# scaleoutsystems/fedn

Measured on AMD Instinct MI355X. Metric: aggregated params/sec (device-resident) — FedAvg 64-client reduce, 100M fp32, higher is better.
Workload: dtype f32

## Files before the change

fedn_amd/_abi.py:

```python
import ctypes
import os
import threading

_HERE = os.path.dirname(os.path.abspath(__file__))
LIB_NAME = "libfedagg.so"
LIB_PATH = os.path.join(_HERE, LIB_NAME)

FA_NONE, FA_F32, FA_F64, FA_BF16, FA_F16, FA_I32, FA_I64 = -1, 0, 1, 2, 3, 4, 5
FA_I8, FA_I16, FA_U8, FA_U16, FA_U32, FA_U64 = 6, 7, 8, 9, 10, 11
FA_OK, FA_EINVAL, FA_EDTYPE, FA_EHIP = 0, 1, 2, 3
FA_ADAM, FA_YOGI, FA_ADAGRAD = 0, 1, 2
FA_PG_FIRST, FA_PG_FINAL = 1, 2
(FA_EW_AXPBY, FA_EW_MUL, FA_EW_DIV, FA_EW_SQRT, FA_EW_SQUARE, FA_EW_SIGN, FA_EW_FILL, FA_EW_POW, FA_EW_IPOW, FA_EW_IFOLD,
 FA_EW_NFOLD) = range(11)
(FA_TUNE_STRIPS, FA_TUNE_UNROLL, FA_TUNE_NT, FA_TUNE_FASTDIV, FA_TUNE_LANETAB, FA_TUNE_GRID, FA_TUNE_READ,
 FA_TUNE_BLOCK, FA_TUNE_SUM_NOSTORE, FA_TUNE_NT_STORE, FA_TUNE_FASTDIV64, FA_TUNE_TILEMAP, FA_TUNE_OPT_NT,
 FA_TUNE_OPT_NOSTORE, FA_TUNE_OPT_STORE, FA_TUNE_OPT_COAL, FA_TUNE_NARROW, FA_TUNE_LDS, FA_TUNE_WPE, FA_TUNE_OPT_MV, FA_TUNE_AUTO_GEOM,
 FA_TUNE_OPT_MIX, FA_TUNE_OPT_BURST, FA_TUNE_OPT_G, FA_TUNE_OPT_WIN_PERIOD, FA_TUNE_OPT_WIN_W, FA_TUNE_OPT_WIN_MODE,
 FA_TUNE_AVG_WIN_PERIOD, FA_TUNE_AVG_WIN_W, FA_TUNE_AVG_WIN_MODE, FA_TUNE_OPT_WIN_PROD,
 FA_TUNE_OPT_QUAD) = range(32)

EXPORTS = {
    "fa_abi_version": (ctypes.c_int, []),
    "fa_last_error": (ctypes.c_char_p, []),
    "fa_last_kernel": (ctypes.c_char_p, []),
    "fa_promote": (ctypes.c_int, [ctypes.c_int, ctypes.c_int]),
    "fa_fedavg_fold": (ctypes.c_int, [
        ctypes.c_void_p, ctypes.c_int,
        ctypes.POINTER(ctypes.c_void_p), ctypes.c_int,
        ctypes.POINTER(ctypes.c_double), ctypes.POINTER(ctypes.c_double), ctypes.c_int,
        ctypes.c_int64, ctypes.c_int, ctypes.c_void_p]),
    "fa_fedavg_fold_host": (ctypes.c_int, [
        ctypes.c_void_p, ctypes.c_int,
        ctypes.POINTER(ctypes.c_void_p), ctypes.c_int,
        ctypes.POINTER(ctypes.c_double), ctypes.POINTER(ctypes.c_double), ctypes.c_int,
        ctypes.c_int64, ctypes.c_int, ctypes.c_void_p]),
    "fa_fedopt_step_host": (ctypes.c_int, [
        ctypes.c_void_p, ctypes.c_int,
        ctypes.POINTER(ctypes.c_void_p), ctypes.c_int,
        ctypes.POINTER(ctypes.c_double), ctypes.POINTER(ctypes.c_double), ctypes.c_int,
        ctypes.c_void_p, ctypes.c_int, ctypes.c_void_p, ctypes.c_int,
        ctypes.c_void_p, ctypes.c_int, ctypes.c_void_p, ctypes.c_void_p, ctypes.c_int,
        ctypes.c_int, ctypes.c_double, ctypes.c_double, ctypes.c_double, ctypes.c_double,
        ctypes.c_int64, ctypes.c_void_p]),
    "fa_fedopt_step": (ctypes.c_int, [
        ctypes.c_void_p, ctypes.c_int,
        ctypes.POINTER(ctypes.c_void_p), ctypes.c_int,
        ctypes.POINTER(ctypes.c_double), ctypes.POINTER(ctypes.c_double), ctypes.c_int,
        ctypes.c_void_p, ctypes.c_int,
        ctypes.c_void_p, ctypes.c_int, ctypes.c_void_p,
        ctypes.c_void_p, ctypes.c_void_p, ctypes.c_void_p,
        ctypes.c_int, ctypes.c_double, ctypes.c_double, ctypes.c_double, ctypes.c_double,
        ctypes.c_int64, ctypes.c_void_p]),
    "fa_fedopt_step_ex": (ctypes.c_int, [
        ctypes.c_void_p, ctypes.c_int,
        ctypes.POINTER(ctypes.c_void_p), ctypes.c_int,
        ctypes.POINTER(ctypes.c_double), ctypes.POINTER(ctypes.c_double), ctypes.c_int,
        ctypes.c_void_p, ctypes.c_int,
        ctypes.c_void_p, ctypes.c_int, ctypes.c_void_p, ctypes.c_int,
        ctypes.c_void_p, ctypes.c_int, ctypes.c_void_p, ctypes.c_void_p, ctypes.c_int,
        ctypes.c_int, ctypes.c_double, ctypes.c_double, ctypes.c_double, ctypes.c_double,
        ctypes.c_int64, ctypes.c_void_p]),
    "fa_weighted_sum": (ctypes.c_int, [
        ctypes.c_void_p, ctypes.c_int,
        ctypes.POINTER(ctypes.c_void_p), ctypes.c_int,
        ctypes.POINTER(ctypes.c_double), ctypes.c_int,
        ctypes.c_int64, ctypes.c_void_p]),
    "fa_running_mean": (ctypes.c_int, [
        ctypes.c_void_p, ctypes.c_int, ctypes.c_void_p,
        ctypes.c_double, ctypes.c_double, ctypes.c_double,
        ctypes.c_int64, ctypes.c_void_p]),
    "fa_elementwise": (ctypes.c_int, [ctypes.c_int, ctypes.c_void_p, ctypes.c_int, ctypes.c_void_p, ctypes.c_int,
                                      ctypes.c_void_p, ctypes.c_int, ctypes.c_double, ctypes.c_double, ctypes.c_int64,
# ... 145 lines not shown
```

fedn_amd/build.py:

```python
import os
import shutil
import subprocess
import sys

HERE = os.path.dirname(os.path.abspath(__file__))
ROOT = os.path.dirname(HERE)
SRC = os.path.join(HERE, "csrc", "fedagg.hip")
HDR = os.path.join(ROOT, "include", "fedagg.h")
OUT = os.path.join(HERE, "libfedagg.so")
PROBE_HDR = os.path.join(ROOT, "include", "fedagg_probe.h")
PROBE_OUT = os.path.join(HERE, "libfedagg_probe.so")
ARCH = os.environ.get("FEDN_AMD_ARCH", "gfx950")

FLAGS = ["-O3", "-std=c++17", "-ffp-contract=off", "-fPIC", "-shared", "-Wall", f"--offload-arch={ARCH}"]


def hipcc():
    for cand in (os.environ.get("HIPCC"), shutil.which("hipcc"), "/opt/rocm/bin/hipcc"):
        if cand and os.path.exists(cand):
            return cand
    raise RuntimeError("hipcc not found")


NPZ_SRC = os.path.join(HERE, "csrc", "npz_codec.cpp")
# ... 11 lines not shown

def build_codec(force=False, verbose=True):
    deps = [d for d in (NPZ_SRC, NPZ_HDR, NPZ_INFLATE, NPZ_SAVEZ, NPZ_PDEFLATE, NPZ_GUARD) if os.path.exists(d)]
    if not force and not _stale(NPZ_OUT, *deps):
        return NPZ_OUT
    cxx = os.environ.get("CXX") or shutil.which("g++") or "g++"
    tmp = NPZ_OUT + ".tmp"
    cmd = [cxx, "-O3", "-std=c++17", "-fPIC", "-shared", "-pthread", "-Wall", "-I", os.path.join(ROOT, "include"),
           "-o", tmp, NPZ_SRC, NPZ_SAVEZ, "-lz"]
    if verbose:
        print(" ".join(cmd), flush=True)
    subprocess.run(cmd, check=True)
    os.replace(tmp, NPZ_OUT)
    return NPZ_OUT


FASTPACK_SRC = os.path.join(HERE, "csrc", "fastpack.c")
FASTPACK_OUT = os.path.join(HERE, "_fastpack.so")


def build_fastpack(force=False, verbose=True):
    if not force and not _stale(FASTPACK_OUT, FASTPACK_SRC):
        return FASTPACK_OUT
    import sysconfig

    import numpy
    cc = os.environ.get("CC") or shutil.which("gcc") or "gcc"
    tmp = FASTPACK_OUT + ".tmp"
    cmd = [cc, "-O2", "-fPIC", "-shared", "-Wall", "-I", sysconfig.get_paths()["include"], "-I", numpy.get_include(),
           "-o", tmp, FASTPACK_SRC]
    if verbose:
        print(" ".join(cmd), flush=True)
    subprocess.run(cmd, check=True)
    os.replace(tmp, FASTPACK_OUT)
    return FASTPACK_OUT


def build(force=False, verbose=True):
    from concurrent.futures import ThreadPoolExecutor
    with ThreadPoolExecutor(4) as ex:
        futs = [ex.submit(build_codec, force, verbose), ex.submit(build_hip, force, verbose),
                ex.submit(build_hip, force, verbose, True), ex.submit(build_fastpack, force, verbose)]
        for f in futs:
            f.result()
    return OUT


def build_hip(force=False, verbose=True, probe=False):
    out = PROBE_OUT if probe else OUT
    deps = (SRC, HDR, PROBE_HDR)
    if not force and not _stale(out, *deps):
        return out
    tmp = out + ".tmp"
    cmd = [hipcc()] + FLAGS + (["-DFEDAGG_PROBES"] if probe else []) + ["-I", os.path.join(ROOT, "include"),
                                                                          "-o", tmp, SRC]
    if verbose:
        print(" ".join(cmd), flush=True)
    subprocess.run(cmd, check=True)
    os.replace(tmp, out)
    return out


if __name__ == "__main__":
    print(build(force="--force" in sys.argv), NPZ_OUT)
```

fedn_amd/csrc/fedagg.hip:

```cpp

#include <hip/hip_runtime.h>
#include <hip/hip_fp16.h>

#include <cmath>
#include <cstdarg>
#include <cstdint>
#include <cstdio>
#include <algorithm>
#include <atomic>
#include <cstring>
#include <type_traits>
#include <vector>

#include "../../include/fedagg.h"
#ifdef FEDAGG_PROBES
#include "../../include/fedagg_probe.h"
#endif

namespace {

thread_local char g_err[512] = "";
thread_local const char* g_kernel = "";

int fail(int code, const char* fmt, ...) {
// ... 562 lines not shown
        };
        auto fold = [&](int kk, const Y (&y)[S][E]) {
            const typename CP::S n = LT ? LaneTable<CP>::rl(lt.n, kk) : tab.n[kk];
            const typename CP::S N = LT ? LaneTable<CP>::rl(lt.N, kk) : tab.N[kk];
            const double r = LT ? LaneTable<CP>::rl(lt.r, kk) : tab.r[kk];
#pragma unroll
            for (int s = 0; s < S; ++s) {
                V yv[E];
#pragma unroll
                for (int e = 0; e < E; ++e) yv[e] = widen<Y, V>(y[s][e]);
                fold_strip<CP, E>(x[s], yv, n, N, r);
            }
        };
        Y a[S][E], b[S][E];
        if (k < K) load(k, a);
        while (k + 1 < K) {
            if constexpr (WIN) {
                if (win_mode >= 2) wait_read_window(period, win_w);
            }
            load(k + 1, b);
            fold(k, a);
            if (k + 2 < K) load(k + 2, a);
            fold(k + 1, b);
            k += 2;
        }
        if (k < K) fold(k, a);
        if constexpr (WIN) wait_write_window(period, win_w);
#pragma unroll
        for (int s = 0; s < S; ++s) {
            X xo[E];
#pragma unroll
            for (int e = 0; e < E; ++e) xo[e] = narrow<X, V>(x[s][e]);
            if constexpr (is_nostore<CP>::value) {
                if (__float_as_uint(x[s][0]) != 0xFFFFFFFFu) continue;
            }
            strip_store<X, E, NTS>(agg + (strip0 + s * BLK) * E, xo);
        }
    }
}

template <typename Y, typename X, class CP, int E, int S, bool INIT, bool INT_FIRST, bool NT, bool LT, int BLK = kBlock,
          int NTS = 0, int MAP = 0>
__global__ void __launch_bounds__(BLK)
k_fedavg_pipe(X* __restrict__ agg, const ClientTable<typename CP::S> tab, const int K, const int64_t P) {
    fedavg_pipe_body<Y, X, CP, E, S, INIT, INT_FIRST, NT, LT, BLK, NTS, MAP>(agg, tab, K, P);
}

template <typename Y, typename X, class CP, int E, int S, bool INIT, bool INT_FIRST, bool NT, bool LT, int BLK, int NTS,
          int MAP>
__global__ void __launch_bounds__(BLK)
k_fedavg_pipe_win(X* __restrict__ agg, const ClientTable<typename CP::S> tab, const int K, const int64_t P,
                  const uint32_t period, const uint32_t win_w, const int win_mode) {
    fedavg_pipe_body<Y, X, CP, E, S, INIT, INT_FIRST, NT, LT, BLK, NTS, MAP, true>(agg, tab, K, P, period, win_w, win_mode);
}

#ifdef FEDAGG_PROBES
template <typename Y, typename X, class CP, int E, int S, bool INIT, bool INT_FIRST, bool NT, bool LT, int BLK, int NTS,
          int MAP, int W>
__global__ void __launch_bounds__(BLK) __attribute__((amdgpu_waves_per_eu(W)))
k_fedavg_pipe_w(X* __restrict__ agg, const ClientTable<typename CP::S> tab, const int K, const int64_t P) {
    fedavg_pipe_body<Y, X, CP, E, S, INIT, INT_FIRST, NT, LT, BLK, NTS, MAP>(agg, tab, K, P);
}
#endif

struct OptScalars {
    double lr, b1, b2, tau, tau2, c1, c2, nc2;
    float b1f, c1f, c2f;
    float b1h, c1h, c2h;
    int opt;
};

struct OptBuffers {
    const void* old;
    void* pg;
    const void* m_in;
    void* m_out;
    const void* v_in;
    void* v_out;
    void* out;
    int m_in_f64;
    int m_out_f64;
    int v_in_f32;
    int v_out_f32;
    int out_f32;
};

template <class PG> __device__ __forceinline__ double mul_pg(double a, double c, float cf, float ch);
template <> __device__ __forceinline__ double mul_pg<CF32>(double a, double, float cf, float) { return (double)((float)a * cf); }
template <> __device__ __forceinline__ double mul_pg<CF64>(double a, double c, float, float) { return a * c; }
template <> __device__ __forceinline__ double mul_pg<CF16>(double a, double, float, float ch) {
    return (double)CF16::rh((float)a * ch);
}

template <class PG> __device__ __forceinline__ typename PG::V pg_sub(typename PG::V y, typename PG::V o) { return y - o; }
template <> __device__ __forceinline__ float pg_sub<CF16>(float y, float o) { return CF16::rh(y - o); }
template <class PG> __device__ __forceinline__ typename PG::V pg_sq(typename PG::V v) { return (typename PG::V)(v * v); }
template <> __device__ __forceinline__ float pg_sq<CF16>(float v) { return CF16::rh(v * v); }

__device__ __forceinline__ double np_sign(double d) {
    return d > 0.0 ? 1.0 : (d < 0.0 ? -1.0 : (d == 0.0 ? 0.0 : d));
}

template <int E, bool SNT = false>
__device__ __forceinline__ void opt_load_state(const OptBuffers& b, const OptScalars& s, int64_t i0, int rem,
                                               double (&mi)[E], double (&v)[E]) {
    const bool full = rem == E;
// ... 971 lines not shown
        for (int j = 0; j < kPushWords; ++j) {
            const int64_t i = base + (int64_t)j * kBlock;
            if (i < n16) v[j] = __builtin_nontemporal_load(src + i);
        }
        for (int d = 0; d < nd; ++d) {
            u32x4* __restrict__ o = t.dst[d];
#pragma unroll
            for (int j = 0; j < kPushWords; ++j) {
                const int64_t i = base + (int64_t)j * kBlock;
                if (i < n16) __builtin_nontemporal_store(v[j], o + i);
            }
        }
    }
}

__global__ void k_push_tail(PushTable t, int nd, const uint8_t* __restrict__ src, int64_t off, int rem) {
    const int b = threadIdx.x;
    if (b < rem)
        for (int d = 0; d < nd; ++d) reinterpret_cast<uint8_t*>(t.dst[d])[off + b] = src[off + b];
}

#ifdef FEDAGG_PROBES
__global__ void __launch_bounds__(kBlock) k_stream_copy(u32x4* __restrict__ dst, const u32x4* __restrict__ src, int64_t n16) {
    const int64_t i = (int64_t)blockIdx.x * kBlock + threadIdx.x;
    if (i < n16) dst[i] = __builtin_nontemporal_load(src + i);
}

constexpr int kReadPerLane = 16;
template <int RPL>
__global__ void __launch_bounds__(kBlock) k_stream_read(const u32x4* __restrict__ src, int64_t n16, u32x4* __restrict__ sink) {
    const int64_t base = (int64_t)blockIdx.x * kBlock * RPL + threadIdx.x;
    u32x4 acc = {0, 0, 0, 0};
#pragma unroll
    for (int j = 0; j < RPL; ++j) {
        const int64_t i = base + (int64_t)j * kBlock;
        if (i < n16) acc ^= __builtin_nontemporal_load(src + i);
    }
    __shared__ u32x4 red[kBlock];
    red[threadIdx.x] = acc;
    __syncthreads();
    if (threadIdx.x == 0) {
        u32x4 r = red[0];
        for (int t = 1; t < kBlock; ++t) r ^= red[t];
        sink[blockIdx.x] = r;
    }
}
#endif

bool aligned16(const void* p) { return (reinterpret_cast<uintptr_t>(p) & 15u) == 0; }

#ifdef FEDAGG_PROBES
struct FedAvgCfg {
    std::atomic<int> strips{4}, unroll{0}, lanetab{0}, grid_per_cu{0}, read_per_lane{16}, block_log{8},
        sum_nostore{0}, nt_store{1}, nt{0}, tilemap{0}, fastdiv{1}, fastdiv64{1}, opt_nt{1}, opt_nostore{0}, opt_store{0}, opt_coal{2}, narrow{1}, lds_kib{0}, wpe{0}, opt_mv{0}, auto_geom{1}, opt_mix{0}, opt_burst{0}, opt_g{0}, opt_win_period{0}, opt_win_w{0}, opt_win_mode{0}, avg_win_period{0}, avg_win_w{0}, avg_win_mode{0}, opt_win_prod{0}, opt_quad{0};
};
FedAvgCfg g_cfg;
int cfg_fastdiv() { return g_cfg.fastdiv.load(std::memory_order_relaxed); }
int cfg_fastdiv64() { return g_cfg.fastdiv64.load(std::memory_order_relaxed); }
int cfg_grid_per_cu() { return g_cfg.grid_per_cu.load(std::memory_order_relaxed); }
#else
constexpr int cfg_fastdiv() { return 1; }
constexpr int cfg_fastdiv64() { return 1; }
constexpr int cfg_grid_per_cu() { return 0; }
#endif

template <typename S>
void fill_table(ClientTable<S>& t, const void* const* ptrs, const double* n, const double* N, int k0, int cnt) {
    for (int j = 0; j < cnt; ++j) {
        t.ptr[j] = ptrs[k0 + j];
        t.n[j] = (S)n[k0 + j];
        t.N[j] = (S)N[k0 + j];
        if constexpr (std::is_same<S, double>::value) {
            const double Nd = N[k0 + j], a = std::fabs(Nd);
            t.r[j] = (cfg_fastdiv64() && a >= 0x1p-60 && a <= 0x1p60) ? 1.0 / Nd : 0.0;
        } else {
            const float Nf = (float)N[k0 + j];
            t.r[j] = (cfg_fastdiv() && Nf != 0.0f && std::fabs(Nf) < 0x1p28f) ? 1.0 / (double)Nf : 0.0;
        }
    }
    for (int j = cnt; j < kMaxK; ++j) {
        t.ptr[j] = nullptr;
        t.n[j] = 0;
        t.N[j] = 0;
        t.r[j] = 0.0;
    }
}

float to_half_value(double v) { return (float)(_Float16)v; }

int64_t grid_for(int64_t P, int E) {
    const int64_t strips = (P + E - 1) / E;
    return (strips + kBlock - 1) / kBlock;
}

int device_cus() {
    int dev = 0, cus = 256;
    if (hipGetDevice(&dev) != hipSuccess ||
        hipDeviceGetAttribute(&cus, hipDeviceAttributeMultiprocessorCount, dev) != hipSuccess)
        cus = 256;
    return cus > 0 ? cus : 256;
}

struct StoreWindow {
    uint32_t period = 0, w = 0;
};
template <typename Y, typename OLD, class PG, bool NT>
StoreWindow opt_store_window(const OptBuffers& b, int K, int64_t P) {
    const bool state = b.m_in_f64 >= 0 || b.v_in;
    if (K < (state ? 32 : 8) || P < ((int64_t)1 << 24)) return {};
    static std::atomic<int> blocks_per_cu{-1};
    int nb = blocks_per_cu.load(std::memory_order_relaxed);
    if (nb < 0) {
        nb = 0;
        if (hipOccupancyMaxActiveBlocksPerMultiprocessor(&nb, k_fedopt_cw<Y, OLD, PG, NT>, kBlock, 0) != hipSuccess) nb = 0;
        blocks_per_cu.store(nb, std::memory_order_relaxed);
    }
    if (nb <= 0) return {};
    const double waves = (double)nb * (kBlock / 64) * device_cus();
    const double m_in = b.m_in_f64 == 1 ? 8 : b.m_in_f64 == 0 ? 4 : b.m_in_f64 < 0 ? 0 : 2;
    const double m_out = b.m_out_f64 == 1 ? 8 : b.m_out_f64 == 0 ? 4 : 2;
    const double rd = (double)K * sizeof(Y) + sizeof(OLD) + m_in + (b.v_in ? (b.v_in_f32 ? 4 : 8) : 0);
    const double wr = (b.out_f32 ? 4 : 8) + (b.v_out_f32 ? 4 : 8) + m_out;
    const double frac = wr / (rd + wr);
    if (frac > 0.25) return {};
    const double period = (state ? 0.35 : 0.65) * waves * 512.0 * (rd + wr) / 6.4e12 * 1e8;
    if (period < 1000 || period > 20000) return {};
    StoreWindow sw;
    sw.period = (uint32_t)period;
    sw.w = (uint32_t)(period * (state ? 0.15 : std::min(0.30, std::max(0.08, 1.15 * frac))));
    return sw;
}


struct AvgWindow {
    uint32_t period = 0, w = 0;
};
template <typename Y, typename X, class CP, int E, int S, bool NT, bool LT, int BLK, int NTS, int MAP>
AvgWindow avg_store_window(int K, int64_t P) {
    if (P < ((int64_t)1 << 24) || K < 2) return {};
    static std::atomic<int> blocks_per_cu{-1};
    int nb = blocks_per_cu.load(std::memory_order_relaxed);
    if (nb < 0) {
        nb = 0;
        if (hipOccupancyMaxActiveBlocksPerMultiprocessor(&nb, k_fedavg_pipe_win<Y, X, CP, E, S, true, false, NT, LT, BLK, NTS, MAP>,
                                                         BLK, 0) != hipSuccess)
            nb = 0;
        blocks_per_cu.store(nb, std::memory_order_relaxed);
    }
    if (nb <= 0) return {};
    if ((double)sizeof(X) / ((double)K * sizeof(Y) + sizeof(X)) > 0.15) return {};
    const double round_bytes = (double)nb * device_cus() * BLK * S * E * ((double)K * sizeof(Y) + sizeof(X));
    const double period = 0.45 * round_bytes / 6.4e12 * 1e8;
    if (period < 500 || period > 20000) return {};
    AvgWindow w;
    w.period = (uint32_t)period;
    w.w = (uint32_t)(0.15 * period);
    return w;
}

template <typename Y, typename X, class CP, int E, int S, bool NT, bool LT, int BLK = kBlock, int NTS = 0, int MAP = 0>
void launch_fedavg_pipe(X* a, const ClientTable<typename CP::S>& tab, int cnt, int64_t P, bool first, bool int_first,
                        hipStream_t st) {
    g_kernel = "k_fedavg_pipe";
    const int64_t strips = (P + E - 1) / E;
    int64_t ntiles = (strips + (int64_t)BLK * S - 1) / ((int64_t)BLK * S);
    if (cfg_grid_per_cu() > 0) {
        if constexpr (MAP != 0) return launch_fedavg_pipe<Y, X, CP, E, S, NT, LT, BLK, NTS, 0>(a, tab, cnt, P, first, int_first, st);
        ntiles = std::min<int64_t>(ntiles, (int64_t)cfg_grid_per_cu() * device_cus());
    }
    const dim3 grid((unsigned)ntiles);
    unsigned shm = 0;
    if constexpr (std::is_same<CP, CF32>::value && std::is_same<X, float>::value &&
                  ((std::is_same<Y, float>::value && S * E == 16) || (std::is_same<Y, bf16>::value && S * E == 32)) &&
                  BLK == kBlock && MAP == 0 && !LT && !NT && NTS == 1) {
        if (first && !int_first && cfg_grid_per_cu() == 0) {
            AvgWindow w = avg_store_window<Y, X, CP, E, S, NT, LT, BLK, NTS, MAP>(cnt, P);
            int wm = 0;
#ifdef FEDAGG_PROBES
            if (g_cfg.avg_win_period < 0 || g_cfg.wpe > 0 || g_cfg.lds_kib > 0) w = AvgWindow{};
            else if (g_cfg.avg_win_period > 0) {
                w = AvgWindow{(uint32_t)g_cfg.avg_win_period.load(), (uint32_t)g_cfg.avg_win_w.load()};
                wm = g_cfg.avg_win_mode.load();
            }
#endif
            if (w.period) {
                g_kernel = "k_fedavg_pipe_win";
                hipLaunchKernelGGL((k_fedavg_pipe_win<Y, X, CP, E, S, true, false, NT, LT, BLK, NTS, MAP>), grid, dim3(BLK), 0, st, a,
                                   tab, cnt, P, w.period, w.w, wm);
                return;
            }
        }
    }
#ifdef FEDAGG_PROBES
    shm = (unsigned)g_cfg.lds_kib * 1024u;
    if constexpr (std::is_same<CP, CF32>::value && std::is_same<X, float>::value && S * E * (int)sizeof(Y) == 64 &&
                  BLK == kBlock && MAP == 0 && !LT && !NT && NTS == 1) {
        if (g_cfg.avg_win_period > 0 && !int_first && !first) {
            const uint32_t wl = (uint32_t)g_cfg.avg_win_period.load(), ww = (uint32_t)g_cfg.avg_win_w.load();
            g_kernel = "k_fedavg_pipe_win";
            hipLaunchKernelGGL((k_fedavg_pipe_win<Y, X, CP, E, S, false, false, NT, LT, BLK, NTS, MAP>), grid, dim3(BLK), shm, st, a, tab,
                               cnt, P, wl, ww, g_cfg.avg_win_mode.load());
            return;
        }
        const int w = g_cfg.wpe;
        if (w > 0 && !int_first) {
#define FA_WPE(W_)                                                                                                      \
    if (w == W_) {                                                                                                      \
        if (first) hipLaunchKernelGGL((k_fedavg_pipe_w<Y, X, CP, E, S, true, false, NT, LT, BLK, NTS, MAP, W_>), grid, dim3(BLK), shm, st, a, tab, cnt, P); \
        else hipLaunchKernelGGL((k_fedavg_pipe_w<Y, X, CP, E, S, false, false, NT, LT, BLK, NTS, MAP, W_>), grid, dim3(BLK), shm, st, a, tab, cnt, P); \
        return;                                                                                                         \
    }
            FA_WPE(5) FA_WPE(6) FA_WPE(8)
#undef FA_WPE
        }
    }
#endif
    if (first && int_first) {
        if constexpr (std::is_integral<Y>::value)
            hipLaunchKernelGGL((k_fedavg_pipe<Y, X, CP, E, S, true, true, NT, LT, BLK, NTS, MAP>), grid, dim3(BLK), shm, st, a, tab, cnt, P);
    } else if (first)
        hipLaunchKernelGGL((k_fedavg_pipe<Y, X, CP, E, S, true, false, NT, LT, BLK, NTS, MAP>), grid, dim3(BLK), shm, st, a, tab, cnt, P);
    else
        hipLaunchKernelGGL((k_fedavg_pipe<Y, X, CP, E, S, false, false, NT, LT, BLK, NTS, MAP>), grid, dim3(BLK), shm, st, a, tab, cnt, P);
}

template <typename Y, typename X, class CP, int E, int S, int U, bool NT>
void launch_fedavg_geom(X* a, const ClientTable<typename CP::S>& tab, int cnt, int64_t P, bool first, bool int_first,
                        hipStream_t st) {
    g_kernel = "k_fedavg";
    const int64_t strips = (P + E - 1) / E;
    const dim3 grid((unsigned)((strips + (int64_t)kBlock * S - 1) / ((int64_t)kBlock * S)));
    if (first && int_first) {
        if constexpr (std::is_integral<Y>::value)
            hipLaunchKernelGGL((k_fedavg<Y, X, CP, E, S, U, true, true, NT>), grid, dim3(kBlock), 0, st, a, tab, cnt, P);
    } else if (first)
        hipLaunchKernelGGL((k_fedavg<Y, X, CP, E, S, U, true, false, NT>), grid, dim3(kBlock), 0, st, a, tab, cnt, P);
    else
        hipLaunchKernelGGL((k_fedavg<Y, X, CP, E, S, U, false, false, NT>), grid, dim3(kBlock), 0, st, a, tab, cnt, P);
}

constexpr int64_t kPipeMinClientBytes = 160ll << 20;

template <typename Y>
inline bool pipe_pays(int64_t P) { return P * (int64_t)sizeof(Y) >= kPipeMinClientBytes; }

template <typename Y, typename X, class CP, int E>
void launch_fedavg_small(X* a, const ClientTable<typename CP::S>& tab, int cnt, int64_t P, bool first, bool int_first,
                         hipStream_t st);

template <class CP> struct is_sf_rule : std::false_type {};
template <typename Y, typename X> struct is_sf_rule<CWSUM<Y, X>> : std::true_type {};
template <typename T_> struct is_sf_rule<CRUN<T_>> : std::true_type {};
// ... 1005 lines not shown
        case FA_TUNE_AUTO_GEOM:
            g_cfg.auto_geom = value ? 1 : 0;
            return FA_OK;
        case FA_TUNE_OPT_MV:
            g_cfg.opt_mv = value ? 1 : 0;
            return FA_OK;
        case FA_TUNE_OPT_MIX:
            g_cfg.opt_mix = value ? 1 : 0;
            return FA_OK;
        case FA_TUNE_OPT_G:
            if (value != 0 && value != 1 && value != 2 && value != 4)
                return fail(FA_EINVAL, "fa_tune: burst-store product probe 0 (off), 1, 2 or 4 tiles per wave");
            g_cfg.opt_g = value;
            return FA_OK;
        case FA_TUNE_OPT_WIN_PERIOD:
            if (value != 0 && value != -1 && (value < 64 || value > (1 << 24)))
                return fail(FA_EINVAL, "fa_tune: store-window period 64 .. 2^24 ticks of 10 ns (0 = the product's own, -1 = none)");
            g_cfg.opt_win_period = value;
            return FA_OK;
        case FA_TUNE_OPT_WIN_W:
            if (value < 0) return fail(FA_EINVAL, "fa_tune: store-window length in ticks >= 0");
            g_cfg.opt_win_w = value;
            return FA_OK;
        case FA_TUNE_OPT_WIN_MODE:
            if (value < 0 || value > 2) return fail(FA_EINVAL, "fa_tune: store-window mode 0, 1 or 2");
            g_cfg.opt_win_mode = value;
            return FA_OK;
        case FA_TUNE_OPT_WIN_PROD:
            if (value < 0 || value > 3)
                return fail(FA_EINVAL, "fa_tune: OPT_WIN_PROD 0 (pattern probe), 1 (k_fedopt_cw), 2 (k_fedopt_cgw), 3 (k_fedopt_cw2)");
            g_cfg.opt_win_prod = value;
            return FA_OK;
        case FA_TUNE_OPT_QUAD:
            g_cfg.opt_quad = value ? 1 : 0;
            return FA_OK;
        case FA_TUNE_AVG_WIN_PERIOD:
            if (value != 0 && value != -1 && (value < 64 || value > (1 << 24)))
                return fail(FA_EINVAL, "fa_tune: store-window period 64 .. 2^24 ticks of 10 ns (0 = the product's own, -1 = none)");
            g_cfg.avg_win_period = value;
            return FA_OK;
        case FA_TUNE_AVG_WIN_W:
            if (value < 0) return fail(FA_EINVAL, "fa_tune: store-window length in ticks >= 0");
            g_cfg.avg_win_w = value;
            return FA_OK;
        case FA_TUNE_AVG_WIN_MODE:
            if (value < 0 || value > 2) return fail(FA_EINVAL, "fa_tune: store-window mode 0, 1 or 2");
            g_cfg.avg_win_mode = value;
            return FA_OK;
        case FA_TUNE_OPT_BURST:
            if (value != 0 && value != 1 && value != 2 && value != 4)
                return fail(FA_EINVAL, "fa_tune: burst-store probe 0 (off), 1, 2 or 4 tiles per wave");
            g_cfg.opt_burst = value;
            return FA_OK;
        case FA_TUNE_WPE:
            if (value != 0 && value != 5 && value != 6 && value != 7 && value != 8)
                return fail(FA_EINVAL, "fa_tune: waves per SIMD 0 (compiler's choice), 5, 6, 7 or 8");
            g_cfg.wpe = value;
            return FA_OK;
        default:
            return fail(FA_EINVAL, "fa_tune: unknown knob %d", knob);
    }
}

int fa_stream_sum(float* out, const float* const* bufs, int K, int64_t P, void* stream) {
    g_err[0] = 0;
    if (K < 1 || K > kMaxK || P < 0 || !out || !bufs) return fail(FA_EINVAL, "fa_stream_sum: bad arguments");
    bool vec = aligned16(out);
    for (int k = 0; k < K; ++k) vec = vec && bufs[k] && aligned16(bufs[k]);
    if (!vec) return fail(FA_EINVAL, "fa_stream_sum: buffers must be 16-B aligned");
    ClientTable<float> tab;
    std::vector<double> ones(K, 1.0);
    fill_table<float>(tab, reinterpret_cast<const void* const*>(bufs), ones.data(), ones.data(), 0, K);
    if (g_cfg.sum_nostore)
        launch_fedavg_pipe<float, float, CADDNW, 4, 4, false, false>(out, tab, K, P, true, false, static_cast<hipStream_t>(stream));
    else if (g_cfg.nt_store == 1)
        launch_fedavg_pipe<float, float, CADD, 4, 4, false, false, kBlock, 1>(out, tab, K, P, true, false, static_cast<hipStream_t>(stream));
    else if (g_cfg.nt_store == 2)
        launch_fedavg_pipe<float, float, CADD, 4, 4, false, false, kBlock, 2>(out, tab, K, P, true, false, static_cast<hipStream_t>(stream));
    else
        launch_fedavg_pipe<float, float, CADD, 4, 4, false, false>(out, tab, K, P, true, false, static_cast<hipStream_t>(stream));
    return check_launch("fa_stream_sum");
}

int fa_stream_copy(void* dst, const void* src, int64_t bytes, void* stream) {
    g_err[0] = 0;
    if (bytes < 0 || (bytes & 15) || !aligned16(dst) || !aligned16(src))
        return fail(FA_EINVAL, "fa_stream_copy: bytes must be a multiple of 16 and buffers 16-B aligned");
    const int64_t n16 = bytes / 16;
    if (!n16) return FA_OK;
    hipLaunchKernelGGL(k_stream_copy, dim3((unsigned)((n16 + kBlock - 1) / kBlock)), dim3(kBlock), 0,
                       static_cast<hipStream_t>(stream), static_cast<u32x4*>(dst), static_cast<const u32x4*>(src), n16);
    return check_launch("fa_stream_copy");
}

int64_t fa_stream_read_blocks(int64_t bytes) {
    const int64_t n16 = bytes / 16;
    const int64_t per = (int64_t)kBlock * kReadPerLane;
    return (n16 + per - 1) / per;
}

int fa_stream_read(const void* src, int64_t bytes, void* sink, void* stream) {
    g_err[0] = 0;
    if (bytes < 0 || (bytes & 15) || !aligned16(src) || !aligned16(sink))
        return fail(FA_EINVAL, "fa_stream_read: bytes must be a multiple of 16 and buffers 16-B aligned");
    const int64_t blocks = fa_stream_read_blocks(bytes);
    if (!blocks) return FA_OK;
// ... 17 lines not shown
```

fedn_amd/ops.py:

```python
import contextlib
import ctypes

import numpy as np
import torch

from . import _abi
from ._abi import FedAggError

_TORCH_TO_FA = {
    torch.float32: _abi.FA_F32,
    torch.float64: _abi.FA_F64,
    torch.bfloat16: _abi.FA_BF16,
    torch.float16: _abi.FA_F16,
    torch.int32: _abi.FA_I32,
    torch.int64: _abi.FA_I64,
    torch.int8: _abi.FA_I8,
    torch.int16: _abi.FA_I16,
    torch.uint8: _abi.FA_U8,
    torch.uint16: _abi.FA_U16,
    torch.uint32: _abi.FA_U32,
    torch.uint64: _abi.FA_U64,
}
_FA_TO_TORCH = {v: k for k, v in _TORCH_TO_FA.items()}
_NP_TO_TORCH = {
# ... 285 lines not shown
        rc = lib.fa_cast(out.data_ptr(), fa_dtype(out), x.data_ptr(), fa_dtype(x), len(ms), _abi.int64_array(ms),
                         _abi.int64_array(mt), st)
    _abi.check(rc)
    return out


def _probe_lib():
    lib = _abi.load()
    if lib is not _abi._probe:
        raise RuntimeError("measurement / tuning entry point: call fedn_amd._abi.use_probe() first "
                           "(libfedagg_probe.so; the product libfedagg.so has no knobs)")
    return lib


def stream_copy(dst, src, stream=None):
    lib = _probe_lib()
    st = _stream_handle(src, stream)
    _abi.check(lib.fa_stream_copy(dst.data_ptr(), src.data_ptr(), src.numel() * src.element_size(), st))


def stream_sum(out, bufs, stream=None):
    lib = _probe_lib()
    st = _stream_handle(out, stream)
    _abi.check(lib.fa_stream_sum(out.data_ptr(), _abi.ptr_array([b.data_ptr() for b in bufs]), len(bufs),
                                 out.numel(), st))


def stream_read(src, sink, stream=None):
    lib = _probe_lib()
    st = _stream_handle(src, stream)
    _abi.check(lib.fa_stream_read(src.data_ptr(), src.numel() * src.element_size(), sink.data_ptr(), st))


def stream_read_sink(src):
    lib = _probe_lib()
    blocks = lib.fa_stream_read_blocks(src.numel() * src.element_size())
    return torch.empty(max(1, blocks) * 16, dtype=torch.uint8, device=src.device)


_KNOBS = {"strips": _abi.FA_TUNE_STRIPS, "unroll": _abi.FA_TUNE_UNROLL, "nt": _abi.FA_TUNE_NT,
          "fastdiv": _abi.FA_TUNE_FASTDIV, "lanetab": _abi.FA_TUNE_LANETAB,
          "grid": _abi.FA_TUNE_GRID, "read": _abi.FA_TUNE_READ,
          "block": _abi.FA_TUNE_BLOCK, "sum_nostore": _abi.FA_TUNE_SUM_NOSTORE,
          "nt_store": _abi.FA_TUNE_NT_STORE, "fastdiv64": _abi.FA_TUNE_FASTDIV64,
          "tilemap": _abi.FA_TUNE_TILEMAP, "opt_nt": _abi.FA_TUNE_OPT_NT, "opt_nostore": _abi.FA_TUNE_OPT_NOSTORE,
          "opt_store": _abi.FA_TUNE_OPT_STORE, "opt_coal": _abi.FA_TUNE_OPT_COAL, "narrow": _abi.FA_TUNE_NARROW,
          "lds": _abi.FA_TUNE_LDS, "wpe": _abi.FA_TUNE_WPE,
          "opt_mv": _abi.FA_TUNE_OPT_MV, "auto_geom": _abi.FA_TUNE_AUTO_GEOM,
          "opt_mix": _abi.FA_TUNE_OPT_MIX, "opt_burst": _abi.FA_TUNE_OPT_BURST,
          "opt_g": _abi.FA_TUNE_OPT_G, "opt_win_period": _abi.FA_TUNE_OPT_WIN_PERIOD, "opt_win_w": _abi.FA_TUNE_OPT_WIN_W,
          "opt_win_mode": _abi.FA_TUNE_OPT_WIN_MODE, "avg_win_period": _abi.FA_TUNE_AVG_WIN_PERIOD,
          "avg_win_w": _abi.FA_TUNE_AVG_WIN_W, "avg_win_mode": _abi.FA_TUNE_AVG_WIN_MODE,
          "opt_win_prod": _abi.FA_TUNE_OPT_WIN_PROD,
          "opt_quad": _abi.FA_TUNE_OPT_QUAD}


def tune(**knobs):
    lib = _probe_lib()
    for k, v in knobs.items():
        _abi.check(lib.fa_tune(_KNOBS[k], int(v)))


_EW = {"axpby": _abi.FA_EW_AXPBY, "mul": _abi.FA_EW_MUL, "div": _abi.FA_EW_DIV, "sqrt": _abi.FA_EW_SQRT,
       "square": _abi.FA_EW_SQUARE, "sign": _abi.FA_EW_SIGN, "fill": _abi.FA_EW_FILL, "pow": _abi.FA_EW_POW,
       "ipow": _abi.FA_EW_IPOW, "ifold": _abi.FA_EW_IFOLD, "nfold": _abi.FA_EW_NFOLD}


def elementwise(op, out, x=None, y=None, a=0.0, b=0.0, stream=None):
    lib = _abi.load()
    P = out.numel()
    _check_dev("out", out, P, None)
    for name, t in (("x", x), ("y", y)):
        if t is not None:
            _check_dev(name, t, P, out.device)
    if P == 0:
        for t in (out, x, y):
            if t is not None:
                fa_dtype(t)
        if op not in _EW:
            raise ValueError(f"unknown elementwise op {op}")
        return out
    with _on(out.device):
        st = _stream_handle(out, stream)
        rc = lib.fa_elementwise(_EW[op], out.data_ptr(), fa_dtype(out), 0 if x is None else x.data_ptr(),
                                fa_dtype(out) if x is None else fa_dtype(x), 0 if y is None else y.data_ptr(),
                                _abi.FA_NONE if y is None else fa_dtype(y), float(a), float(b), P, st)
    _abi.check(rc)
    return out


def norm1(x, matrix, stream=None):
    lib = _abi.load()
    if not x.is_contiguous():
        raise ValueError("norm1: x must be contiguous")
    rows, cols = (x.shape[0], x.shape[1]) if matrix else (1, x.numel())
    work = torch.empty(max(1, int(lib.fa_norm1_work(rows, cols, int(matrix)))), dtype=torch.float64, device=x.device)
    out = torch.empty((), dtype=torch.float64, device=x.device)
    with _on(x.device):
        st = _stream_handle(x, stream)
        rc = lib.fa_norm1(out.data_ptr(), x.data_ptr(), fa_dtype(x), rows, cols, int(matrix), work.data_ptr(), st)
    _abi.check(rc)
    return out



def ipc_handle(t):
    import ctypes
# ... 167 lines not shown
```

include/fedagg_probe.h:

```cpp
#ifndef FEDAGG_PROBE_H
#define FEDAGG_PROBE_H

#include "fedagg.h"

#ifdef __cplusplus
extern "C" {
#endif

int fa_stream_copy(void* dst, const void* src, int64_t bytes, void* stream);
int fa_stream_sum(float* out, const float* const* bufs, int K, int64_t P, void* stream);

enum fa_tune_knob { FA_TUNE_STRIPS = 0, FA_TUNE_UNROLL = 1, FA_TUNE_NT = 2, FA_TUNE_FASTDIV = 3, FA_TUNE_LANETAB = 4,
                    FA_TUNE_GRID = 5, FA_TUNE_READ = 6 ,
                    FA_TUNE_BLOCK = 7 ,
                    FA_TUNE_SUM_NOSTORE = 8 ,
                    FA_TUNE_NT_STORE = 9 ,
                    FA_TUNE_FASTDIV64 = 10 ,
                    FA_TUNE_TILEMAP = 11 ,
                    FA_TUNE_OPT_NT = 12 ,
                    FA_TUNE_OPT_NOSTORE = 13 ,
                    FA_TUNE_OPT_STORE = 14 ,
                    FA_TUNE_OPT_COAL = 15 ,
                    FA_TUNE_NARROW = 16 ,
                    FA_TUNE_LDS = 17 ,
                    FA_TUNE_WPE = 18 ,
                    FA_TUNE_OPT_MV = 19 ,
                    FA_TUNE_AUTO_GEOM = 20 ,
                    FA_TUNE_OPT_MIX = 21 ,
                    FA_TUNE_OPT_BURST = 22 ,
                    FA_TUNE_OPT_G = 23 ,
                    FA_TUNE_OPT_WIN_PERIOD = 24 ,
                    FA_TUNE_OPT_WIN_W = 25 ,
                    FA_TUNE_OPT_WIN_MODE = 26 ,
                    FA_TUNE_AVG_WIN_PERIOD = 27 ,
                    FA_TUNE_AVG_WIN_W = 28,
                    FA_TUNE_AVG_WIN_MODE = 29,
                    FA_TUNE_OPT_WIN_PROD = 30 ,
                    FA_TUNE_OPT_QUAD = 31  };
int fa_tune(int knob, int value);
int64_t fa_stream_read_blocks(int64_t bytes);
int fa_stream_read(const void* src, int64_t bytes, void* sink, void* stream);

#ifdef __cplusplus
}
#endif

#endif
```

Measured before the change: 1489 billion.

## Add rolling-refill FedAvg fold kernel for large client counts with tuned store window

Adds a new FedAvg fold body that keeps one client's strips in flight and refills each strip's buffer right after folding it, replacing the ping-pong double-buffer body for f32 inputs when K >= 48. The aim is smoother memory-level parallelism and fewer stalls between clients in the bandwidth-bound reduce. The roll kernel uses its own store-window period (a smaller fraction of the round bytes, with a higher cap). The build now also captures compiler kernel-resource remarks into a file, and a probe knob selects the fold body. Risk: different register pressure and occupancy, and a new tuned window heuristic.

```diff
diff --git a/fedn_amd/_abi.py b/fedn_amd/_abi.py
--- a/fedn_amd/_abi.py
+++ b/fedn_amd/_abi.py
@@ -18,7 +18,7 @@
  FA_TUNE_OPT_NOSTORE, FA_TUNE_OPT_STORE, FA_TUNE_OPT_COAL, FA_TUNE_NARROW, FA_TUNE_LDS, FA_TUNE_WPE, FA_TUNE_OPT_MV, FA_TUNE_AUTO_GEOM,
  FA_TUNE_OPT_MIX, FA_TUNE_OPT_BURST, FA_TUNE_OPT_G, FA_TUNE_OPT_WIN_PERIOD, FA_TUNE_OPT_WIN_W, FA_TUNE_OPT_WIN_MODE,
  FA_TUNE_AVG_WIN_PERIOD, FA_TUNE_AVG_WIN_W, FA_TUNE_AVG_WIN_MODE, FA_TUNE_OPT_WIN_PROD,
- FA_TUNE_OPT_QUAD) = range(32)
+ FA_TUNE_OPT_QUAD, FA_TUNE_AVG_BODY) = range(33)
 
 EXPORTS = {
     "fa_abi_version": (ctypes.c_int, []),
diff --git a/fedn_amd/build.py b/fedn_amd/build.py
--- a/fedn_amd/build.py
+++ b/fedn_amd/build.py
@@ -87,14 +87,52 @@
     if not force and not _stale(out, *deps):
         return out
     tmp = out + ".tmp"
-    cmd = [hipcc()] + FLAGS + (["-DFEDAGG_PROBES"] if probe else []) + ["-I", os.path.join(ROOT, "include"),
+    cmd = [hipcc()] + FLAGS + (["-DFEDAGG_PROBES"] if probe else []) + [RESOURCE_FLAG, "-I", os.path.join(ROOT, "include"),
                                                                           "-o", tmp, SRC]
     if verbose:
         print(" ".join(cmd), flush=True)
-    subprocess.run(cmd, check=True)
+    p = subprocess.run(cmd, stderr=subprocess.PIPE, text=True)
+    import re
+    remarks, rest, quoted = [], [], False
+    for line in p.stderr.splitlines(keepends=True):
+        if RESOURCE_FLAG in line:
+            remarks.append(line)
+            quoted = True
+        elif not (quoted and re.match(r"\s*\d*\s*\|", line)):
+            rest.append(line)
+            quoted = False
+    sys.stderr.write("".join(rest))
+    if p.returncode:
+        raise subprocess.CalledProcessError(p.returncode, cmd)
+    with open(resources_path(probe), "w") as f:
+        f.writelines(remarks)
     os.replace(tmp, out)
     return out
 
 
+RESOURCE_FLAG = "-Rpass-analysis=kernel-resource-usage"
+
+
+def resources_path(probe=False):
+    return (PROBE_OUT if probe else OUT) + ".resources.txt"
+
+
+def kernel_resources(text):
+    import re
+    fields = {"VGPRs": "vgprs", "AGPRs": "agprs", "TotalSGPRs": "sgprs", "ScratchSize [bytes/lane]": "scratch",
+              "Occupancy [waves/SIMD]": "occupancy"}
+    res, cur = {}, None
+    for line in text.splitlines():
+        m = re.search(r"remark: (?:\S+: )?\s*([A-Za-z][A-Za-z /\[\]]*?): (\S+) \[" + re.escape(RESOURCE_FLAG), line)
+        if not m:
+            continue
+        key, val = m.group(1).strip(), m.group(2)
+        if key == "Function Name":
+            cur = res.setdefault(val, {})
+        elif cur is not None and key in fields and val.isdigit():
+            cur[fields[key]] = int(val)
+    return res
+
+
 if __name__ == "__main__":
     print(build(force="--force" in sys.argv), NPZ_OUT)
diff --git a/fedn_amd/csrc/fedagg.hip b/fedn_amd/csrc/fedagg.hip
--- a/fedn_amd/csrc/fedagg.hip
+++ b/fedn_amd/csrc/fedagg.hip
@@ -638,6 +638,82 @@
 k_fedavg_pipe_win(X* __restrict__ agg, const ClientTable<typename CP::S> tab, const int K, const int64_t P,
                   const uint32_t period, const uint32_t win_w, const int win_mode) {
     fedavg_pipe_body<Y, X, CP, E, S, INIT, INT_FIRST, NT, LT, BLK, NTS, MAP, true>(agg, tab, K, P, period, win_w, win_mode);
+}
+
+template <typename Y, typename X, class CP, int E, int S, bool INIT, bool NT, int BLK, int NTS, int MAP, bool WIN = false>
+__device__ __forceinline__ void fedavg_roll_body(X* __restrict__ agg, const ClientTable<typename CP::S>& tab, const int K,
+                                                 const int64_t P, const uint32_t period = 0, const uint32_t win_w = 0,
+                                                 const int win_mode = 0) {
+    using V = typename CP::V;
+    const int64_t ntiles = ((P + E - 1) / E + (int64_t)BLK * S - 1) / ((int64_t)BLK * S);
+    for (int64_t t = blockIdx.x; t < ntiles; t += gridDim.x) {
+        const int64_t tile = map_tile<MAP>(t, ntiles);
+        const int64_t strip0 = tile * (BLK * S) + threadIdx.x;
+        if ((strip0 + (int64_t)(S - 1) * BLK) * E + E > P) {
+            k_fedavg_tail<Y, X, CP, E, S, INIT, false, BLK>(agg, tab, K, P, strip0);
+            continue;
+        }
+        if constexpr (WIN) {
+            if (win_mode >= 1) wait_read_window(period, win_w);
+        }
+        V x[S][E];
+        int k = 0;
+#pragma unroll
+        for (int s = 0; s < S; ++s)
+            k = strip_start<Y, X, CP, E, INIT, false, NT>(x[s], agg, tab, (strip0 + s * BLK) * E, E);
+        const int64_t tile_b = tile * ((int64_t)BLK * S * E * sizeof(Y));
+        const uint32_t lane_b = (uint32_t)threadIdx.x * (uint32_t)(E * sizeof(Y));
+        auto load = [&](int kk, int s, Y (&y)[E]) {
+            const char* yp = static_cast<const char*>(tab.ptr[kk]) + tile_b + (int64_t)s * (BLK * E * sizeof(Y));
+            uint32_t off = lane_b;
+            asm volatile("" : "+v"(off));
+            strip_load<Y, E, NT>(reinterpret_cast<const Y*>(yp + off), y);
+        };
+        Y y[S][E];
+        if (k < K) {
+#pragma unroll
+            for (int s = 0; s < S; ++s) load(k, s, y[s]);
+        }
+        for (; k < K; ++k) {
+            const bool more = k + 1 < K;
+            if constexpr (WIN) {
+                if (win_mode >= 2 && more) wait_read_window(period, win_w);
+            }
+            const typename CP::S n = tab.n[k], N = tab.N[k];
+            const double r = tab.r[k];
+#pragma unroll
+            for (int s = 0; s < S; ++s) {
+                V yv[E];
+#pragma unroll
+                for (int e = 0; e < E; ++e) yv[e] = widen<Y, V>(y[s][e]);
+                fold_strip<CP, E>(x[s], yv, n, N, r);
+#pragma unroll
+                for (int e = 0; e < E; ++e) asm volatile("" : "+v"(x[s][e]));
+                if (more) load(k + 1, s, y[s]);
+            }
+        }
+        if constexpr (WIN) wait_write_window(period, win_w);
+#pragma unroll
+        for (int s = 0; s < S; ++s) {
+            X xo[E];
+#pragma unroll
+            for (int e = 0; e < E; ++e) xo[e] = narrow<X, V>(x[s][e]);
+            strip_store<X, E, NTS>(agg + (strip0 + s * BLK) * E, xo);
+        }
+    }
+}
+
+template <typename Y, typename X, class CP, int E, int S, bool INIT, bool NT, int BLK, int NTS, int MAP>
+__global__ void __launch_bounds__(BLK)
+k_fedavg_roll(X* __restrict__ agg, const ClientTable<typename CP::S> tab, const int K, const int64_t P) {
+    fedavg_roll_body<Y, X, CP, E, S, INIT, NT, BLK, NTS, MAP>(agg, tab, K, P);
+}
+
+template <typename Y, typename X, class CP, int E, int S, bool INIT, bool NT, int BLK, int NTS, int MAP>
+__global__ void __launch_bounds__(BLK)
+k_fedavg_roll_win(X* __restrict__ agg, const ClientTable<typename CP::S> tab, const int K, const int64_t P,
+                  const uint32_t period, const uint32_t win_w, const int win_mode) {
+    fedavg_roll_body<Y, X, CP, E, S, INIT, NT, BLK, NTS, MAP, true>(agg, tab, K, P, period, win_w, win_mode);
 }
 
 #ifdef FEDAGG_PROBES
@@ -1715,17 +1791,42 @@
 #ifdef FEDAGG_PROBES
 struct FedAvgCfg {
     std::atomic<int> strips{4}, unroll{0}, lanetab{0}, grid_per_cu{0}, read_per_lane{16}, block_log{8},
-        sum_nostore{0}, nt_store{1}, nt{0}, tilemap{0}, fastdiv{1}, fastdiv64{1}, opt_nt{1}, opt_nostore{0}, opt_store{0}, opt_coal{2}, narrow{1}, lds_kib{0}, wpe{0}, opt_mv{0}, auto_geom{1}, opt_mix{0}, opt_burst{0}, opt_g{0}, opt_win_period{0}, opt_win_w{0}, opt_win_mode{0}, avg_win_period{0}, avg_win_w{0}, avg_win_mode{0}, opt_win_prod{0}, opt_quad{0};
+        sum_nostore{0}, nt_store{1}, nt{0}, tilemap{0}, fastdiv{1}, fastdiv64{1}, opt_nt{1}, opt_nostore{0}, opt_store{0}, opt_coal{2}, narrow{1}, lds_kib{0}, wpe{0}, opt_mv{0}, auto_geom{1}, opt_mix{0}, opt_burst{0}, opt_g{0}, opt_win_period{0}, opt_win_w{0}, opt_win_mode{0}, avg_win_period{0}, avg_win_w{0}, avg_win_mode{0}, opt_win_prod{0}, opt_quad{0}, avg_body{0};
 };
 FedAvgCfg g_cfg;
 int cfg_fastdiv() { return g_cfg.fastdiv.load(std::memory_order_relaxed); }
 int cfg_fastdiv64() { return g_cfg.fastdiv64.load(std::memory_order_relaxed); }
 int cfg_grid_per_cu() { return g_cfg.grid_per_cu.load(std::memory_order_relaxed); }
+int cfg_avg_body() { return g_cfg.avg_body.load(std::memory_order_relaxed); }
 #else
 constexpr int cfg_fastdiv() { return 1; }
 constexpr int cfg_fastdiv64() { return 1; }
 constexpr int cfg_grid_per_cu() { return 0; }
+constexpr int cfg_avg_body() { return 0; }
 #endif
+
+template <typename Y> constexpr int kAvgRollMinK = 0;
+template <> constexpr int kAvgRollMinK<float> = 48;
+template <typename Y>
+constexpr bool avg_roll_built() {
+#ifdef FEDAGG_PROBES
+    return true;
+#else
+    return kAvgRollMinK<Y> > 0;
+#endif
+}
+template <typename Y>
+inline bool avg_product_roll(int K) { return kAvgRollMinK<Y> > 0 && K >= kAvgRollMinK<Y>; }
+
+inline const char* avg_kernel_name(bool win, [[maybe_unused]] bool roll) {
+#ifdef FEDAGG_PROBES
+    if (cfg_avg_body() != 0) {
+        if (win) return roll ? "k_fedavg_pipe_win/roll" : "k_fedavg_pipe_win/pingpong";
+        return roll ? "k_fedavg_pipe/roll" : "k_fedavg_pipe/pingpong";
+    }
+#endif
+    return win ? "k_fedavg_pipe_win" : "k_fedavg_pipe";
+}
 
 template <typename S>
 void fill_table(ClientTable<S>& t, const void* const* ptrs, const double* n, const double* N, int k0, int cnt) {
@@ -1798,23 +1899,28 @@
 struct AvgWindow {
     uint32_t period = 0, w = 0;
 };
-template <typename Y, typename X, class CP, int E, int S, bool NT, bool LT, int BLK, int NTS, int MAP>
+constexpr double kAvgPingPeriod = 0.45, kAvgRollPeriod = 0.10;
+template <typename Y, typename X, class CP, int E, int S, bool NT, bool LT, int BLK, int NTS, int MAP, bool ROLL = false>
 AvgWindow avg_store_window(int K, int64_t P) {
     if (P < ((int64_t)1 << 24) || K < 2) return {};
     static std::atomic<int> blocks_per_cu{-1};
     int nb = blocks_per_cu.load(std::memory_order_relaxed);
     if (nb < 0) {
         nb = 0;
-        if (hipOccupancyMaxActiveBlocksPerMultiprocessor(&nb, k_fedavg_pipe_win<Y, X, CP, E, S, true, false, NT, LT, BLK, NTS, MAP>,
-                                                         BLK, 0) != hipSuccess)
-            nb = 0;
+        hipError_t e;
+        if constexpr (ROLL)
+            e = hipOccupancyMaxActiveBlocksPerMultiprocessor(&nb, k_fedavg_roll_win<Y, X, CP, E, S, true, NT, BLK, NTS, MAP>, BLK, 0);
+        else
+            e = hipOccupancyMaxActiveBlocksPerMultiprocessor(&nb, k_fedavg_pipe_win<Y, X, CP, E, S, true, false, NT, LT, BLK, NTS, MAP>,
+                                                             BLK, 0);
+        if (e != hipSuccess) nb = 0;
         blocks_per_cu.store(nb, std::memory_order_relaxed);
     }
     if (nb <= 0) return {};
     if ((double)sizeof(X) / ((double)K * sizeof(Y) + sizeof(X)) > 0.15) return {};
     const double round_bytes = (double)nb * device_cus() * BLK * S * E * ((double)K * sizeof(Y) + sizeof(X));
-    const double period = 0.45 * round_bytes / 6.4e12 * 1e8;
-    if (period < 500 || period > 20000) return {};
+    const double period = (ROLL ? kAvgRollPeriod : kAvgPingPeriod) * round_bytes / 6.4e12 * 1e8;
+    if (period < 500 || period > (ROLL ? 48000 : 20000)) return {};
     AvgWindow w;
     w.period = (uint32_t)period;
     w.w = (uint32_t)(0.15 * period);
@@ -1836,23 +1942,51 @@
     if constexpr (std::is_same<CP, CF32>::value && std::is_same<X, float>::value &&
                   ((std::is_same<Y, float>::value && S * E == 16) || (std::is_same<Y, bf16>::value && S * E == 32)) &&
                   BLK == kBlock && MAP == 0 && !LT && !NT && NTS == 1) {
-        if (first && !int_first && cfg_grid_per_cu() == 0) {
-            AvgWindow w = avg_store_window<Y, X, CP, E, S, NT, LT, BLK, NTS, MAP>(cnt, P);
+        if (!int_first && cfg_grid_per_cu() == 0) {
+            AvgWindow w{};
             int wm = 0;
+            [[maybe_unused]] bool roll = false;
+            if constexpr (avg_roll_built<Y>()) {
+                roll = cfg_avg_body() == 2 || (cfg_avg_body() == 0 && first && avg_product_roll<Y>(cnt));
+                if (first && roll) {
+                    w = avg_store_window<Y, X, CP, E, S, NT, LT, BLK, NTS, MAP, true>(cnt, P);
+                    if (cfg_avg_body() == 0 && !w.period) roll = false;
+                }
+            }
+            if (first && !roll) w = avg_store_window<Y, X, CP, E, S, NT, LT, BLK, NTS, MAP>(cnt, P);
 #ifdef FEDAGG_PROBES
-            if (g_cfg.avg_win_period < 0 || g_cfg.wpe > 0 || g_cfg.lds_kib > 0) w = AvgWindow{};
-            else if (g_cfg.avg_win_period > 0) {
+            const bool occ_probe = g_cfg.wpe > 0 || g_cfg.lds_kib > 0;
+            if (occ_probe) roll = false;
+            if (g_cfg.avg_win_period < 0 || occ_probe) w = AvgWindow{};
+            else if (g_cfg.avg_win_period > 0 && (first || roll)) {
                 w = AvgWindow{(uint32_t)g_cfg.avg_win_period.load(), (uint32_t)g_cfg.avg_win_w.load()};
                 wm = g_cfg.avg_win_mode.load();
             }
 #endif
-            if (w.period) {
-                g_kernel = "k_fedavg_pipe_win";
+            if constexpr (avg_roll_built<Y>()) {
+                if (roll) {
+                    g_kernel = avg_kernel_name(w.period != 0, true);
+                    if (w.period && first)
+                        hipLaunchKernelGGL((k_fedavg_roll_win<Y, X, CP, E, S, true, NT, BLK, NTS, MAP>), grid, dim3(BLK), 0, st, a, tab,
+                                           cnt, P, w.period, w.w, wm);
+                    else if (w.period)
+                        hipLaunchKernelGGL((k_fedavg_roll_win<Y, X, CP, E, S, false, NT, BLK, NTS, MAP>), grid, dim3(BLK), 0, st, a, tab,
+                                           cnt, P, w.period, w.w, wm);
+                    else if (first)
+                        hipLaunchKernelGGL((k_fedavg_roll<Y, X, CP, E, S, true, NT, BLK, NTS, MAP>), grid, dim3(BLK), 0, st, a, tab, cnt, P);
+                    else
+                        hipLaunchKernelGGL((k_fedavg_roll<Y, X, CP, E, S, false, NT, BLK, NTS, MAP>), grid, dim3(BLK), 0, st, a, tab, cnt, P);
+                    return;
+                }
+            }
+            if (first && w.period) {
+                g_kernel = avg_kernel_name(true, false);
                 hipLaunchKernelGGL((k_fedavg_pipe_win<Y, X, CP, E, S, true, false, NT, LT, BLK, NTS, MAP>), grid, dim3(BLK), 0, st, a,
                                    tab, cnt, P, w.period, w.w, wm);
                 return;
             }
         }
+        g_kernel = avg_kernel_name(false, false);
     }
 #ifdef FEDAGG_PROBES
     shm = (unsigned)g_cfg.lds_kib * 1024u;
@@ -1860,7 +1994,7 @@
                   BLK == kBlock && MAP == 0 && !LT && !NT && NTS == 1) {
         if (g_cfg.avg_win_period > 0 && !int_first && !first) {
             const uint32_t wl = (uint32_t)g_cfg.avg_win_period.load(), ww = (uint32_t)g_cfg.avg_win_w.load();
-            g_kernel = "k_fedavg_pipe_win";
+            g_kernel = avg_kernel_name(true, false);
             hipLaunchKernelGGL((k_fedavg_pipe_win<Y, X, CP, E, S, false, false, NT, LT, BLK, NTS, MAP>), grid, dim3(BLK), shm, st, a, tab,
                                cnt, P, wl, ww, g_cfg.avg_win_mode.load());
             return;
@@ -2972,6 +3106,10 @@
                 return fail(FA_EINVAL, "fa_tune: burst-store probe 0 (off), 1, 2 or 4 tiles per wave");
             g_cfg.opt_burst = value;
             return FA_OK;
+        case FA_TUNE_AVG_BODY:
+            if (value < 0 || value > 2) return fail(FA_EINVAL, "fa_tune: fold body 0 (the product's choice), 1 (ping-pong) or 2 (rolling refill)");
+            g_cfg.avg_body = value;
+            return FA_OK;
         case FA_TUNE_WPE:
             if (value != 0 && value != 5 && value != 6 && value != 7 && value != 8)
                 return fail(FA_EINVAL, "fa_tune: waves per SIMD 0 (compiler's choice), 5, 6, 7 or 8");
diff --git a/fedn_amd/ops.py b/fedn_amd/ops.py
--- a/fedn_amd/ops.py
+++ b/fedn_amd/ops.py
@@ -361,7 +361,7 @@
           "opt_win_mode": _abi.FA_TUNE_OPT_WIN_MODE, "avg_win_period": _abi.FA_TUNE_AVG_WIN_PERIOD,
           "avg_win_w": _abi.FA_TUNE_AVG_WIN_W, "avg_win_mode": _abi.FA_TUNE_AVG_WIN_MODE,
           "opt_win_prod": _abi.FA_TUNE_OPT_WIN_PROD,
-          "opt_quad": _abi.FA_TUNE_OPT_QUAD}
+          "opt_quad": _abi.FA_TUNE_OPT_QUAD, "avg_body": _abi.FA_TUNE_AVG_BODY}
 
 
 def tune(**knobs):
diff --git a/include/fedagg_probe.h b/include/fedagg_probe.h
--- a/include/fedagg_probe.h
+++ b/include/fedagg_probe.h
@@ -36,7 +36,8 @@
                     FA_TUNE_AVG_WIN_W = 28,
                     FA_TUNE_AVG_WIN_MODE = 29,
                     FA_TUNE_OPT_WIN_PROD = 30 ,
-                    FA_TUNE_OPT_QUAD = 31  };
+                    FA_TUNE_OPT_QUAD = 31 ,
+                    FA_TUNE_AVG_BODY = 32  };
 int fa_tune(int knob, int value);
 int64_t fa_stream_read_blocks(int64_t bytes);
 int fa_stream_read(const void* src, int64_t bytes, void* sink, void* stream);
```

After: 1503 billion, median of 6. Within noise of the previous version (+1.0%).
